# glennhickey/teHmm

Hardware: AMD Instinct MI355X
Metric: genome positions/sec (Viterbi+posterior), 35 states x 10 tracks (higher is better)
Workload: dtype f64

## Files before the change

### tehmm_amd/csrc/tehmm_coop.hip.h

```cpp
#pragma once
#include "tehmm_kernels.hip.h"

namespace tehmm {

typedef double d2v __attribute__((ext_vector_type(2)));
typedef __attribute__((address_space(3))) const d2v lds_cd2;
__device__ __forceinline__ lds_cd2 *lds_row(const double *row) {
  unsigned a = (unsigned)(size_t)(__attribute__((address_space(3))) const double *)row;
  asm volatile("v_mov_b32 %0, %1" : "=v"(a) : "v"(a));
  return (lds_cd2 *)(size_t)a;
}

template <int NT>
__device__ __forceinline__ void rep_rows(double v, double (&r)[(NT + 15) / 16]) {
  const unsigned lo = __double2loint(v), hi = __double2hiint(v);
  const auto a = __builtin_amdgcn_permlane32_swap(lo, lo, false, false);
  const auto b = __builtin_amdgcn_permlane32_swap(hi, hi, false, false);
  const auto c = __builtin_amdgcn_permlane16_swap(a[0], a[0], false, false);
  const auto d = __builtin_amdgcn_permlane16_swap(b[0], b[0], false, false);
  r[0] = __hiloint2double((int)d[0], (int)c[0]);
  if constexpr (NT > 16) r[1] = __hiloint2double((int)d[1], (int)c[1]);
  if constexpr (NT > 32) {
    const auto e = __builtin_amdgcn_permlane16_swap(a[1], a[1], false, false);
    const auto f = __builtin_amdgcn_permlane16_swap(b[1], b[1], false, false);
    r[2] = __hiloint2double((int)f[0], (int)e[0]);
    if constexpr (NT > 48) r[3] = __hiloint2double((int)f[1], (int)e[1]);
  }
}
template <int L>
__device__ __forceinline__ double bcast(double v) {
  return __longlong_as_double(
      __builtin_amdgcn_mov_dpp(__double_as_longlong(v), 0x150 + L, 0xf, 0xf, true));
}
template <int F, int NT>
struct BcastAdd {
  static __device__ __forceinline__ void run(const double (&r)[(NT + 15) / 16], const double (&ltc)[NT],
                                             double (&x)[NT]) {
    x[F] = bcast<F & 15>(r[F >> 4]) + ltc[F];
    BcastAdd<F + 1, NT>::run(r, ltc, x);
  }
};
template <int NT>
struct BcastAdd<NT, NT> {
  static __device__ __forceinline__ void run(const double (&)[(NT + 15) / 16], const double (&)[NT],
                                             double (&)[NT]) {}
};
template <int F, int NT>
struct BcastFma {
  static __device__ __forceinline__ void run(const double (&r)[(NT + 15) / 16], const double (&ac)[NT],
                                             double (&s)[4]) {
    asm volatile("v_fmac_f64_dpp %0, %1, %2 row_newbcast:%3 row_mask:0xf bank_mask:0xf"
                 : "+v"(s[F & 3])
                 : "v"(r[F >> 4]), "v"(ac[F]), "n"(F & 15));
    BcastFma<F + 1, NT>::run(r, ac, s);
  }
};
template <int NT>
struct BcastFma<NT, NT> {
  static __device__ __forceinline__ void run(const double (&)[(NT + 15) / 16], const double (&)[NT],
                                             double (&)[4]) {}
};

__device__ __forceinline__ double exp_nonpos(double y) {
  const double k = rint(y * 1.4426950408889634);
  double r = fma(k, -6.93147180369123816490e-01, y);
  r = fma(k, -1.90821492927058770002e-10, r);
  double p = 1.6059043836821613e-10;
  p = fma(p, r, 2.08767569878681e-09);
  p = fma(p, r, 2.505210838544172e-08);
  p = fma(p, r, 2.755731922398589e-07);
  p = fma(p, r, 2.7557319223985893e-06);
  p = fma(p, r, 2.48015873015873e-05);
  p = fma(p, r, 1.984126984126984e-04);
  p = fma(p, r, 1.388888888888889e-03);
  p = fma(p, r, 8.333333333333333e-03);
  p = fma(p, r, 4.1666666666666664e-02);
  p = fma(p, r, 1.6666666666666666e-01);
  p = fma(p, r, 0.5);
  p = fma(p, r, 1.0);
  p = fma(p, r, 1.0);
  const double res = ldexp(p, (int)k);
  return y < -1100.0 ? 0.0 : res;
}

template <int NT>
__device__ __forceinline__ void emis_rows(const EmisTab &e, const double *ltab, int64_t gpos,
                                          double (&x)[NT]) {
  const uint32_t *row = e.obs32 + gpos * e.KPW;
#pragma unroll
  for (int j = 0; j < NT; ++j) x[j] = 0.0;
  uint32_t wn = row[0];
  for (int d = 0; d < e.KPW; ++d) {
    const uint32_t w = wn;
    if (d + 1 < e.KPW) wn = row[d + 1];
#pragma unroll
    for (int bb = 0; bb < 4; ++bb) {
      const int k = 4 * d + bb;
      if (k < e.K) {
        const int sym = (int)((w >> (8 * bb)) & 0xffu);
        const bool inr = sym < e.rowcnt[k];
        const int lb = e.ldsbase[k];
        if (lb >= 0) {
          lds_cd2 *tr = (lds_cd2 *)(size_t)((unsigned)(size_t)(
              __attribute__((address_space(3))) const double *)ltab +
              (unsigned)((inr ? lb + sym : e.lds_zero) * NT * 8));
#pragma unroll
          for (int jj = 0; jj < NT / 2; ++jj) {
            const d2v v = tr[jj];
            x[2 * jj] += v.x;
            x[2 * jj + 1] += v.y;
          }
        } else {
          const double2 *tr = (const double2 *)(e.tab + (int64_t)(inr ? e.rowbase[k] + sym : e.zero_row) * NT);
#pragma unroll
          for (int jj = 0; jj < NT / 2; ++jj) {
            const double2 v = tr[jj];
            x[2 * jj] += v.x;
            x[2 * jj + 1] += v.y;
          }
        }
      }
    }
  }
#pragma unroll
  for (int j = 0; j < NT; ++j) x[j] *= e.normalize;
  if (e.ratios) {
    const double r = e.ratios[gpos];
#pragma unroll
    for (int j = 0; j < NT; ++j) x[j] *= r;
  }
}

template <int NT, bool LINEAR, bool ASCENDING, bool TRATIO>
__device__ __forceinline__ void emis_block(const EmisTab &e, const double *ltab, int64_t gbase,
                                           int np, int lane, int N, bool &seen, int *dead,
                                           const double *ltdiag, const double *tratios,
                                           double *ring, int RS, double *ms) {
  const bool act = lane < np;
  const int64_t gpos = gbase + (act ? lane : np - 1);
  double x[NT];
  emis_rows<NT>(e, ltab, gpos, x);
  double m = x[0];
#pragma unroll
  for (int j = 1; j < NT; ++j) m = fmax(m, j < N ? x[j] : -INFINITY);
  const bool good = m > -1e20;
  bool zero;
  if (ASCENDING) {
    const unsigned long long gm = __ballot(good && act);
    const int first = gm ? __ffsll((long long)gm) - 1 : 64;
    zero = !seen && lane < first;
    if (!good && !zero && act && dead) *dead = 1;
    if (gm) seen = true;
  } else {
    zero = !good;
  }
  if (zero) {
#pragma unroll
    for (int j = 0; j < NT; ++j) x[j] = 0.0;
    m = 0.0;
  }
  if (TRATIO) {
    const double r = tratios[gpos];
    if (r > 1.) {
      m = -INFINITY;
#pragma unroll
      for (int j = 0; j < NT; ++j) {
        x[j] += ltdiag[j] * (r - 1.);
        m = fmax(m, j < N ? x[j] : -INFINITY);
      }
    }
  }
  if (act) {
    double *dst = ring + lane * RS;
    if (LINEAR) {
#pragma unroll
      for (int j = 0; j < NT; ++j) dst[j] = j < N ? exp_nonpos(x[j] - m) : 0.0;
      ms[lane] = m;
    } else {
#pragma unroll
      for (int j = 0; j < NT; ++j) dst[j] = x[j];
    }
  }
}

__device__ __forceinline__ void stage_emis_table(const EmisTab &e, double *ltab, int NT) {
  const int n = e.lds_rows * NT;
  for (int i = threadIdx.x; i < n; i += blockDim.x) ltab[i] = e.ltab_src[i];
}

template <int NT, int CPB, bool RATIO>
__global__ __launch_bounds__(256) __attribute__((amdgpu_waves_per_eu(1, 1)))
void k_vit_coop(IntervalTab iv, EmisTab em, int N, const double *g_lt, const double *g_ltT,
                const double *g_pi, const double *tratios, uint8_t *tb, int *last_state, double *logprob) {
  extern __shared__ double sm[];
  constexpr int RS = NT + 1;
  constexpr int VS = NT + 2;
  double *bring = sm;
  double *Vring = bring + 3 * CPB * RS;
  double *ltab = Vring + 2 * (CPB + 1) * VS;
  const int lane = threadIdx.x & 63;
  const int w = threadIdx.x >> 6;
  const int id = iv.order[blockIdx.x];
  const int64_t T = iv.len[id];
  const int64_t p0 = iv.pos0[id];
  if (T <= 0) return;
  stage_emis_table(em, ltab, NT);
  const int jl = min(lane, NT - 1);
  const bool live = lane < N;
  ST_DECL;
  __syncthreads();
  const int64_t nb = (T + CPB - 1) / CPB;
  if (w == 0) {
    double ltc[NT];
#pragma unroll
    for (int f = 0; f < NT; ++f) ltc[f] = live ? g_lt[f * NT + jl] : -INFINITY;
    const double ltd = live ? g_lt[jl * NT + jl] : 0.0;
    const double lt00 = g_lt[0];
    const double pij = live ? g_pi[jl] : -INFINITY;
    const int vslot = lane < NT ? lane : NT + 1;
    double vcur = -INFINITY;
    for (int64_t it = 0; it < nb + 2; ++it) {
      ST_BEGIN;
      const int64_t bn = it - 1;
      if (bn >= 0 && bn < nb) {
        const int np = (int)min((int64_t)CPB, T - bn * CPB);
        double *Vr = Vring + (bn & 1) * (CPB + 1) * VS;
        const double *br = bring + (bn % 3) * CPB * RS;
        if (bn > 0) Vr[vslot] = vcur;
        for (int p = 0; p < np; ++p) {
          const int64_t t = bn * CPB + p;
          const double b = br[p * RS + jl];
          double r = 0.0;
          if (RATIO) r = tratios[p0 + t];
          double v;
          if (t == 0) {
            v = pij + b;
            if (RATIO && r > 1.) v += ltd * (r - 1.);
          } else {
            double rr[(NT + 15) / 16];
            rep_rows<NT>(vcur, rr);
            double x[NT];
            BcastAdd<0, NT>::run(rr, ltc, x);
            double c0 = x[0] + b;
            x[0] = -INFINITY;
#pragma unroll
            for (int n = NT; n > 1; n = (n + 1) / 2) {
#pragma unroll
              for (int i = 0; i < n / 2; ++i) x[i] = fmax(x[i], x[i + (n + 1) / 2]);
            }
            if (RATIO) {
              c0 += ltd * r;
              if (lane == 0) c0 -= lt00;
            }
            double c1 = x[0] + b;
            if (RATIO && r > 1.) c1 += ltd * (r - 1.);
            v = c1 > c0 ? c1 : c0;
          }
          vcur = v;
          Vr[(p + 1) * VS + vslot] = v;
        }
      }
      ST_ADD(st_a);
      __syncthreads();
      ST_ADD(st_c);
    }
    ST_FLUSH(w);
    double *scratch = Vring;
    if (lane < NT) scratch[lane] = vcur;
    __builtin_amdgcn_wave_barrier();
    if (lane == 0) {
      int last = 0;
      double m = scratch[0];
      if (m == m) {
        for (int j = 1; j < N; ++j) {
          double x = scratch[j];
          if (x != x) { last = j; break; }
          if (x > m) { m = x; last = j; }
        }
      }
      last_state[id] = last;
      logprob[id] = scratch[last];
    }
  } else if (w == 1) {
    bool seen = false;
    for (int64_t it = 0; it < nb + 2; ++it) {
      ST_BEGIN;
#ifdef TEHMM_DBG_NOEMIS
      if (it < 3) {
#else
      if (it < nb) {
#endif
        const int np = (int)min((int64_t)CPB, T - it * CPB);
        emis_block<NT, false, true, false>(em, ltab, p0 + it * CPB, np, lane, N, seen, nullptr,
                                           nullptr, nullptr, bring + (it % 3) * CPB * RS, RS,
                                           nullptr);
      }
      ST_ADD(st_a);
      __syncthreads();
      ST_ADD(st_c);
    }
    ST_FLUSH(w);
  } else {
    const int half = (N + 1) / 2;
    const int to_lo = (w - 2) * half, to_hi = min(N, to_lo + half);
    const double lt00 = g_lt[0];
    for (int64_t it = 0; it < nb + 2; ++it) {
      ST_BEGIN;
      const int64_t ba = it - 2;
#ifdef TEHMM_DBG_NOARGS
      if (ba >= 0 && ba < 1) {
#else
      if (ba >= 0 && ba < nb) {
#endif
        const int np = (int)min((int64_t)CPB, T - ba * CPB);
        const double *Vr = Vring + (ba & 1) * (CPB + 1) * VS;
        const double *br = bring + (ba % 3) * CPB * RS;
        const int pl = lane < np ? lane : 0;
        const int64_t t = ba * CPB + pl;
        const bool actp = lane < np && t > 0;
        lds_cd2 *vp = lds_row(Vr + pl * VS);
        d2v pv[NT / 2];
#pragma unroll
        for (int f2 = 0; f2 < NT / 2; ++f2) pv[f2] = vp[f2];
        const double *vnext = Vr + (pl + 1) * VS;
        const double *brow = br + pl * RS;
        double r = 0.0;
        if (RATIO) r = tratios[p0 + t];
        const bool rg = RATIO && r > 1.;
        for (int to = to_lo; to < to_hi; ++to) {
          const double *lc = g_ltT + to * NT;
          const double vt = vnext[to];
          const double b = brow[to];
          double c[NT];
#pragma unroll
          for (int f2 = 0; f2 < NT / 2; ++f2) {
            c[2 * f2] = (pv[f2].x + lc[2 * f2]) + b;
            c[2 * f2 + 1] = (pv[f2].y + lc[2 * f2 + 1]) + b;
          }
          if (RATIO) {
            const double ld = lc[to];
            c[0] += ld * r;
            if (to == 0) c[0] -= lt00;
            const double addr = rg ? ld * (r - 1.) : 0.0;
#pragma unroll
            for (int f = 1; f < NT; ++f) c[f] += addr;
          }
          int arg = 0;
#pragma unroll
          for (int f = NT - 1; f >= 1; --f) arg = c[f] == vt ? f : arg;
          arg = c[0] == vt ? 0 : arg;
          if (actp) tb[(p0 + t) * NT + to] = (uint8_t)arg;
        }
      }
      ST_ADD(st_b);
      __syncthreads();
      ST_ADD(st_c);
    }
    ST_FLUSH(w);
  }
}

template <int NT, int CPB, bool TRATIO>
__global__ __launch_bounds__(256) __attribute__((amdgpu_waves_per_eu(1, 1)))
void k_fb_coop(IntervalTab iv, EmisTab em, int N, const double *g_A, const double *g_lt,
               const double *g_pi, const double *tratios, double *alpha, double *beta,
               double *fwd_logprob, int *dead_flag, double *wrows, int *escale) {
  extern __shared__ double sm[];
  constexpr int RS = NT + 1;
  double *ringF = sm;
  double *ringB = ringF + 2 * CPB * RS;
  double *msF = ringB + 2 * CPB * RS;
  double *msB = msF + 2 * CPB;
  double *xF = msB + 2 * CPB;
  double *xB = xF + 2 * NT;
  double *ltdv = xB + 2 * NT;
  double *ltab = ltdv + NT;
  const int lane = threadIdx.x & 63;
  const int w = threadIdx.x >> 6;
  const int id = iv.order[blockIdx.x];
  const int64_t T = iv.len[id];
  const int64_t p0 = iv.pos0[id];
  if (T <= 0) return;
  const int jl = min(lane, NT - 1);
  const bool live = lane < N;
  if (threadIdx.x < NT) ltdv[threadIdx.x] = g_lt[threadIdx.x * NT + threadIdx.x];
  stage_emis_table(em, ltab, NT);
  ST_DECL;
  __syncthreads();
  const int64_t nb = (T + CPB - 1) / CPB;
  if (w == 0) {
    double ac[NT];
#pragma unroll
    for (int i = 0; i < NT; ++i) ac[i] = live ? g_A[i * NT + jl] : (lane == NT - 1 ? 1.0 : 0.0);
    double *al = alpha + iv.out0[id] * N;
    int *es = escale ? escale + iv.out0[id] : nullptr;
    double Ecum = 0.0, Mcum = 0.0, a = 0.0;
    for (int64_t it = 0; it < nb + 1; ++it) {
      ST_BEGIN;
      const int64_t bn = it - 1;
      if (bn >= 0) {
        const int np = (int)min((int64_t)CPB, T - bn * CPB);
        const double *br = ringF + (bn & 1) * CPB * RS;
        const double *mr = msF + (bn & 1) * CPB;
        for (int p = 0; p < np; ++p) {
          const int64_t t = bn * CPB + p;
          const double bh = br[p * RS + jl];
          Mcum += mr[p];
          if (t == 0) {
            a = live ? exp(g_pi[jl]) * bh : 0.0;
          } else {
            double rr[(NT + 15) / 16];
            rep_rows<NT>(a, rr);
            double sacc[4] = {0.0, 0.0, 0.0, 0.0};
            asm volatile("s_nop 1" ::: "memory");
            BcastFma<0, NT>::run(rr, ac, sacc);
            const double ssum = (sacc[0] + sacc[1]) + (sacc[2] + sacc[3]);
            const int e = ((__builtin_amdgcn_readlane(__double2hiint(ssum), NT - 1) >> 20) & 0x7ff) - 1022;
            a = live ? ldexp(ssum * bh, -e) : 0.0;
            Ecum += (double)e;
            if (es && lane == 0) es[t] = e;
          }
          if (live) al[t * N + lane] = a;
        }
      }
      ST_ADD(st_a);
      __syncthreads();
      ST_ADD(st_c);
    }
    ST_FLUSH(w);
    double tot = wave_sum_f64(live ? a : 0.0);
    if (lane == 0) fwd_logprob[id] = log(tot) + Ecum * 0.6931471805599453 + Mcum;
  } else if (w == 1) {
    double ac[NT];
#pragma unroll
    for (int j = 0; j < NT; ++j) ac[j] = live ? g_A[jl * NT + j] : (lane == NT - 1 ? 1.0 : 0.0);
    double *be = beta + iv.out0[id] * N;
    double *wr = wrows ? wrows + iv.out0[id] * N : nullptr;
    double bt = 0.0, wv = 0.0;
    for (int64_t it = 0; it < nb + 1; ++it) {
      ST_BEGIN;
      const int64_t bn = it - 1;
      if (bn >= 0) {
        const int64_t uhi = T - bn * CPB;
        const int64_t ulo = max((int64_t)0, uhi - CPB);
        const double *br = ringB + (bn & 1) * CPB * RS;
        for (int64_t u = uhi - 1; u >= ulo; --u) {
          const double bh = br[(int)(u - ulo) * RS + jl];
          if (u == T - 1) {
            bt = live ? 1.0 : 0.0;
          } else {
            double rr[(NT + 15) / 16];
            rep_rows<NT>(wv, rr);
            double sacc[4] = {0.0, 0.0, 0.0, 0.0};
            asm volatile("s_nop 1" ::: "memory");
            BcastFma<0, NT>::run(rr, ac, sacc);
            const double ssum = (sacc[0] + sacc[1]) + (sacc[2] + sacc[3]);
            const int e = ((__builtin_amdgcn_readlane(__double2hiint(ssum), NT - 1) >> 20) & 0x7ff) - 1022;
            bt = live ? ldexp(ssum, -e) : 0.0;
          }
          if (live) be[u * N + lane] = bt;
          wv = live ? bh * bt : 0.0;
          if (wr && live) wr[u * N + lane] = wv;
        }
      }
      ST_ADD(st_a);
      __syncthreads();
      ST_ADD(st_c);
    }
    ST_FLUSH(w);
  } else if (w == 2) {
    bool seen = false;
    for (int64_t it = 0; it < nb + 1; ++it) {
      ST_BEGIN;
      if (it < nb) {
        const int np = (int)min((int64_t)CPB, T - it * CPB);
        emis_block<NT, true, true, TRATIO>(em, ltab, p0 + it * CPB, np, lane, N, seen, dead_flag + id,
                                           ltdv, tratios, ringF + (it & 1) * CPB * RS, RS,
                                           msF + (it & 1) * CPB);
      }
      ST_ADD(st_a);
      __syncthreads();
      ST_ADD(st_c);
    }
    ST_FLUSH(w);
  } else {
    for (int64_t it = 0; it < nb + 1; ++it) {
      ST_BEGIN;
      if (it < nb) {
        const int64_t uhi = T - it * CPB;
        const int64_t ulo = max((int64_t)0, uhi - CPB);
// ... 200 lines not shown
```

### tehmm_amd/csrc/tehmm_lane.hip.h

```cpp
#pragma once
#include "tehmm_spec.hip.h"

namespace tehmm {

typedef __attribute__((address_space(4))) const double const_f64;
#define TEHMM_TG(f, o, NT) ((((o) >> 2) * (NT) + (f)) * 4 + ((o) & 3))



template <int NT>
__global__ __launch_bounds__(256) void k_emis_lane(IntervalTab iv, EmisTab em, LaneGeom lg, int N,
                                                   double *B, double *BH, double *MS, float *B32) {
  extern __shared__ double emis_ltab[];
  stage_emis_table(em, emis_ltab, NT);
  __syncthreads();
  const int lane = threadIdx.x & 63;
  const int g = blockIdx.x * 4 + (threadIdx.x >> 6);
  if (g >= lg.n_groups) return;
  const int64_t item = (int64_t)g * 64 + lane;
  const bool valid = item < lg.n_items;
  const int id = valid ? lg.item_iv[item] : 0;
  const int64_t t0 = valid ? lg.item_t0[item] : 0;
  const int64_t T = iv.len[id], p0 = iv.pos0[id];
  const int len = valid ? (int)min((int64_t)lg.L, T - t0) : 0;
// ... 663 lines not shown
    vec_out(vi.end);
    if (QUANT) {
      vi.ntie[item] = nt;
      vi.bad[item] = (bad || nt > TEHMM_LANE_MAXTI) ? 1 : 0;
      vi.piecemin[item * (TEHMM_LANE_MAXTI + 1) + min(nt, TEHMM_LANE_MAXTI)] = pmin;
    } else {
      const double g1 = vec_max();
      vi.gain[item] = bad ? __longlong_as_double(0x7ff8000000000000LL) : g1 - g0;
    }
  }
}

template <int NT>
__global__ __launch_bounds__(256) void k_vit_stitch(IntervalTab iv, LaneGeom lg, VitChunks vc, VitItems vi,
                                                    int N, int soft = 0) {
  const int lane = threadIdx.x & 63;
  const int c = blockIdx.x * 4 + (threadIdx.x >> 6);
  if (c >= vc.n) return;
  if (vc.e[c] == TEHMM_SPEC_NONE) {
    if (lane == 0) { vc.ok[c] = 0; vc.ntie[c] = 0; vc.offend[c] = 0.0; if (vc.tsoft) { vc.tsoft[c] = 0u; vc.tpar[c] = 0u; } }
    return;
  }
  unsigned softmask = 0u, parmask = 0u;
  const double uinv = ldexp(1.0, 52 - vc.e[c]);
  auto odd_mult = [&](double x) { const double q = x * uinv * 0.5; return q != trunc(q); };
  const int id = vc.iv[c];
  const int64_t ct0 = vc.t0[c];
  const int L = lg.L, SUB = vc.CS / L, R = L / TEHMM_VROW;
  const int64_t item0 = lg.ifirst[id] + ct0 / L;
  const bool live = lane < N;
  const int jl = min(lane, NT - 1);
  auto at = [&](const double *p, int64_t item) { return p[((((item >> 6) * NT) + jl) << 6) + (item & 63)]; };
  double off = 0.0, off_end = 0.0, segmin = INFINITY;
  int nT = 0;
  bool okc = true;
  for (int k = 0; k < SUB; ++k) {
    const int64_t item = item0 + k;
    okc = okc && vi.bad[item] == 0;
    off = off_end;
    if (k > 0) {
      const double a = at(vi.pre, item), bp = at(vi.end, item - 1);
      const bool both_dead = a == -INFINITY && bp == -INFINITY;
      const double d = bp - a;
      const double d0 = wave_max_live((both_dead || !live) ? -INFINITY : d, live);
      const bool same = __all(!live || both_dead || d == d0) && d0 == d0 && d0 > -INFINITY && d0 < INFINITY;
      if (same) {
        off = off_end + d0;
      } else {
        if (nT < TEHMM_SPEC_MAXT) {
          if (lane == 0) {
            vc.ties[(int64_t)c * TEHMM_SPEC_MAXT + nT] = k * L;
            vc.segmin[(int64_t)c * (TEHMM_SPEC_MAXT + 1) + nT] = segmin;
          }
          if (lane < NT) vc.tierows[((int64_t)c * TEHMM_SPEC_MAXT + nT) * NT + lane] = bp + off_end;
        }
        ++nT;
        off = 0.0;
        segmin = INFINITY;
      }
    }
    const int nti = min(vi.ntie[item], TEHMM_LANE_MAXTI);
    const int first_tie = nti > 0 ? vi.ties[item * TEHMM_LANE_MAXTI] : L;
    if (off != 0.0 && lane < NT) {
      for (int m = 0; m < R && (soft || TEHMM_VROW * m + TEHMM_VROW - 1 < first_tie); ++m)
        vc.rows[((int64_t)c * (vc.CS / TEHMM_VROW) + k * R + m) * NT + lane] += off;
    }
    segmin = fmin(segmin, vi.piecemin[item * (TEHMM_LANE_MAXTI + 1)] + off);
    for (int i = 0; i < nti; ++i) {
      if (nT < TEHMM_SPEC_MAXT) {
        if (lane == 0) {
          vc.ties[(int64_t)c * TEHMM_SPEC_MAXT + nT] = k * L + vi.ties[item * TEHMM_LANE_MAXTI + i];
          vc.segmin[(int64_t)c * (TEHMM_SPEC_MAXT + 1) + nT] = segmin;
        }
        if (lane < NT)
          vc.tierows[((int64_t)c * TEHMM_SPEC_MAXT + nT) * NT + lane] =
              vi.tierows[(item * TEHMM_LANE_MAXTI + i) * NT + lane] + ((i == 0 || soft) ? off : 0.0);
        if (soft) {
          softmask |= 1u << nT;
          if (odd_mult(off)) parmask |= 1u << nT;
        }
      }
      ++nT;
      segmin = vi.piecemin[item * (TEHMM_LANE_MAXTI + 1) + i + 1] + (soft ? off : 0.0);
    }
    off_end = (nti > 0 && !soft) ? 0.0 : off;
  }
  if (lane == 0) {
    vc.segmin[(int64_t)c * (TEHMM_SPEC_MAXT + 1) + min(nT, TEHMM_SPEC_MAXT)] = segmin;
    vc.ntie[c] = nT;
    vc.ok[c] = (okc && nT <= TEHMM_SPEC_MAXT) ? 1 : 0;
    vc.offend[c] = off_end;
    if (vc.tsoft) { vc.tsoft[c] = softmask; vc.tpar[c] = parmask; }
  }
}

template <int NT>
__global__ __launch_bounds__(256) void k_vit_links(IntervalTab iv, LaneGeom lg, VitChunks vc, VitItems vi, int N) {
  const int lane = threadIdx.x & 63;
  const int c = blockIdx.x * 4 + (threadIdx.x >> 6);
  if (c >= vc.n) return;
  const int id = vc.iv[c];
  bool cand = c > vc.first[id] && vc.e[c] != TEHMM_SPEC_NONE && vc.e[c - 1] == vc.e[c] && vc.ok[c] != 0 &&
              vc.ok[c - 1] != 0;
  int link = 0;
  double lk = 0.0;
  if (cand) {
    const int L = lg.L;
    const int64_t item0 = lg.ifirst[id] + vc.t0[c] / L;
    const bool live = lane < N;
    const int jl = min(lane, NT - 1);
    auto at = [&](const double *p, int64_t item) { return p[((((item >> 6) * NT) + jl) << 6) + (item & 63)]; };
    const double a = at(vi.pre, item0);
    const double bp = at(vi.end, item0 - 1) + vc.offend[c - 1];
    const bool both_dead = a == -INFINITY && bp == -INFINITY;
    const double d = bp - a;
    const double d0 = wave_max_live((both_dead || !live) ? -INFINITY : d, live);
    const bool same = __all(!live || both_dead || d == d0) && d0 == d0 && d0 > -INFINITY && d0 < INFINITY;
    if (same && vi.bad[item0 - 1] == 0 && vi.bad[item0] == 0) {
      link = 1;
      lk = d0;
    }
  }
  if (lane == 0) {
    vc.clink[c] = link;
    vc.clk[c] = lk;
  }
}


struct VitRunMap {
  int stop;
  int64_t target, sel;
  double acc, mn;
};
struct VitRunMap2 {
  VitRunMap m[2];
  int hout[2];
};
__device__ __forceinline__ VitRunMap2 vit_run_compose(const VitRunMap2 &a, const VitRunMap2 &b) {
  VitRunMap2 r;
#pragma unroll
  for (int h = 0; h < 2; ++h) {
    if (a.m[h].stop) {
      r.m[h] = a.m[h];
      r.hout[h] = 0;
    } else {
      const int h2 = a.hout[h];
      const VitRunMap &bb = h2 ? b.m[1] : b.m[0];
      r.m[h].stop = bb.stop;
      r.m[h].target = bb.target;
      r.m[h].sel = bb.sel;
      r.m[h].acc = a.m[h].acc + bb.acc;
      r.m[h].mn = fmin(a.m[h].mn, a.m[h].acc + bb.mn);
      r.hout[h] = h2 ? b.hout[1] : b.hout[0];
    }
  }
  return r;
}
__global__ __launch_bounds__(64) void k_vit_runs(VitChunks vc, int n_iv) {
  const int lane = threadIdx.x;
  const int id = blockIdx.x;
  if (id >= n_iv) return;
  const int64_t c0 = vc.first[id], c1 = vc.first[id + 1];
  const int64_t nc = vc.n;
  VitRunMap2 carry;
  carry.m[0] = carry.m[1] = VitRunMap{0, 0, 0, 0.0, INFINITY};
  carry.hout[0] = 0;
  carry.hout[1] = 1;
  for (int64_t hi = c1; hi > c0; hi -= 64) {
    const int64_t c = hi - 64 + lane;
    const bool in = c >= c0;
    VitRunMap2 m;
    m.m[0] = m.m[1] = VitRunMap{0, 0, 0, 0.0, INFINITY};
    m.hout[0] = 0;
    m.hout[1] = 1;
    if (in) {
      const double *sm = vc.segmin + c * (TEHMM_SPEC_MAXT + 1);
      const bool linked_next = c + 1 < c1 && vc.clink[c + 1] != 0;
      const int nt = min(vc.ntie[c], TEHMM_SPEC_MAXT);
      const unsigned soft = vc.tsoft ? vc.tsoft[c] : 0u, par = vc.tsoft ? vc.tpar[c] : 0u;
      int kodd = 0;
      if (linked_next) {
        const double q = vc.clk[c + 1] * ldexp(1.0, 52 - vc.e[c]) * 0.5;
        kodd = q != trunc(q);
      }
#pragma unroll
      for (int h = 0; h < 2; ++h) {
        int kh = -1;
        double mn = sm[0];
        for (int k = 0; k < nt; ++k) {
          if (!((soft >> k) & 1u) || (int)((par >> k) & 1u) != h) { kh = k; break; }
          mn = fmin(mn, sm[k + 1]);
        }
        if (kh >= 0) m.m[h] = VitRunMap{1, vc.t0[c] + vc.ties[c * TEHMM_SPEC_MAXT + kh], 2 * (64 * c + kh), 0.0, mn};
        else if (linked_next) m.m[h] = VitRunMap{0, 0, 0, vc.clk[c + 1], mn};
        else m.m[h] = VitRunMap{1, vc.t0[c] + vc.CS, 2 * (64 * c) + 1, 0.0, mn};
        m.hout[h] = h ^ kodd;
      }
    }
#pragma unroll
    for (int d = 1; d < 64; d <<= 1) {
      VitRunMap2 o;
#pragma unroll
      for (int h = 0; h < 2; ++h) {
        o.m[h].stop = __shfl_down(m.m[h].stop, d);
        o.m[h].target = __shfl_down(m.m[h].target, d);
        o.m[h].sel = __shfl_down(m.m[h].sel, d);
        o.m[h].acc = __shfl_down(m.m[h].acc, d);
        o.m[h].mn = __shfl_down(m.m[h].mn, d);
        o.hout[h] = __shfl_down(m.hout[h], d);
      }
      if (lane + d < 64) m = vit_run_compose(m, o);
    }
    m = vit_run_compose(m, carry);
    if (in) {
#pragma unroll
      for (int h = 0; h < 2; ++h) {
        vc.rtarget[h * nc + c] = m.m[h].target;
        vc.rsel[h * nc + c] = m.m[h].sel;
        vc.racc[h * nc + c] = m.m[h].acc;
        vc.rmn[h * nc + c] = m.m[h].mn;
      }
    }
#pragma unroll
    for (int h = 0; h < 2; ++h) {
      carry.m[h].stop = __shfl(m.m[h].stop, 0);
      carry.m[h].target = __shfl(m.m[h].target, 0);
      carry.m[h].sel = __shfl(m.m[h].sel, 0);
      carry.m[h].acc = __shfl(m.m[h].acc, 0);
      carry.m[h].mn = __shfl(m.m[h].mn, 0);
      carry.hout[h] = __shfl(m.hout[h], 0);
    }
  }
}


typedef float lane_f2 __attribute__((ext_vector_type(2)));
typedef __attribute__((address_space(4))) const lane_f2 const_f2;

template <int NT>
__global__ __launch_bounds__(256) void k_vit_gain_lane(IntervalTab iv, LaneGeom lg, int N, int CS, int Wu,
                                                       const float *__restrict__ tabf,
                                                       const float *__restrict__ B32, double *gain) {
  const int lane = threadIdx.x & 63;
  const int g = blockIdx.x * 4 + (threadIdx.x >> 6);
  if (g >= lg.n_groups) return;
  const int L = lg.L;
  const int64_t item = (int64_t)g * 64 + lane;
  const bool valid = item < lg.n_items;
  const int id = valid ? lg.item_iv[item] : 0;
  const int64_t t0 = valid ? lg.item_t0[item] : 0;
  const int64_t T = iv.len[id];
  const int64_t ct0 = (t0 / CS) * CS;
  const bool run = valid && ct0 > 0 && ct0 + CS <= T;
  if (!__any(run)) return;
  const int64_t nb = run ? item - 1 : item;
  lane_f2 W[NT / 2];
#pragma unroll
  for (int j = 0; j < NT / 2; ++j)
    W[j] = (lane_f2){2 * j < N ? 0.f : -INFINITY, 2 * j + 1 < N ? 0.f : -INFINITY};
  bool bad = false;
  auto vec_max = [&]() {
    float mx = -INFINITY;
#pragma unroll
    for (int j = 0; j < NT / 2; ++j) mx = fmaxf(mx, fmaxf(W[j].x, W[j].y));
    return mx;
  };
  float g0 = 0.f;
  for (int s = -Wu; s < L; ++s) {
    if (s == 0) g0 = vec_max();
    const float *bp = B32 + (s < 0 ? lane_row(lg, NT, nb, L + s) : lane_row(lg, NT, item, s));
    float b[NT];
#pragma unroll
    for (int j = 0; j < NT; ++j) b[j] = bp[(int64_t)j << 6];
    bad = bad | (b[0] != b[0]);
    int z = 0;
    asm volatile("" : "+s"(z));
    const_f2 *tp = (const_f2 *)(size_t)tabf + z;
    lane_f2 x[NT / 2];
#pragma unroll
    for (int op = 0; op < NT / 2; ++op) {
      lane_f2 acc = (lane_f2){W[0].x, W[0].x} + tp[op * NT];
#pragma unroll
      for (int f = 1; f < NT; ++f) {
        const float wf = (f & 1) ? W[f >> 1].y : W[f >> 1].x;
        acc = __builtin_elementwise_max(acc, (lane_f2){wf, wf} + tp[op * NT + f]);
      }
      x[op] = acc;
    }
#pragma unroll
    for (int j = 0; j < NT / 2; ++j) W[j] = x[j] + (lane_f2){b[2 * j], b[2 * j + 1]};
  }
  if (run) gain[item] = bad ? __longlong_as_double(0x7ff8000000000000LL) : (double)vec_max() - (double)g0;
}

template <int NT, bool RATIO = false>
#ifndef TEHMM_EMIS_WAVES
#define TEHMM_EMIS_WAVES 2
#endif
__global__ __launch_bounds__(256) __attribute__((amdgpu_waves_per_eu(TEHMM_EMIS_WAVES, TEHMM_EMIS_WAVES))) void k_emis_gain_lane(IntervalTab iv, EmisTab em, LaneGeom lg, int N, int CS, int Wu,
                                                        const float *__restrict__ tabf, double *B, double *gain,
                                                        const double *__restrict__ ratios = nullptr) {
  extern __shared__ double emis_ltab[];
  stage_emis_table(em, emis_ltab, NT);
  __syncthreads();
  const int lane = threadIdx.x & 63;
  const int g = blockIdx.x * 4 + (threadIdx.x >> 6);
  if (g >= lg.n_groups) return;
  const int L = lg.L;
  const int64_t item = (int64_t)g * 64 + lane;
  const bool valid = item < lg.n_items;
  const int id = valid ? lg.item_iv[item] : 0;
  const int64_t t0 = valid ? lg.item_t0[item] : 0;
  const int64_t T = iv.len[id], p0 = iv.pos0[id];
  const int len = valid ? (int)min((int64_t)L, T - t0) : 0;
  const int maxlen = wave_max_i32(len);
  const int64_t ct0 = (t0 / CS) * CS;
  const bool run = valid && ct0 > 0 && ct0 + CS <= T;
  const int s_first = __any(run) ? -Wu : 0;
  const double qnan = __longlong_as_double(0x7ff8000000000000LL);
  lane_f2 W[NT / 2];
#pragma unroll
  for (int j = 0; j < NT / 2; ++j)
    W[j] = (lane_f2){2 * j < N ? 0.f : -INFINITY, 2 * j + 1 < N ? 0.f : -INFINITY};
  bool bad = false;
  auto vec_max = [&]() {
    float mx = -INFINITY;
#pragma unroll
    for (int j = 0; j < NT / 2; ++j) mx = fmaxf(mx, fmaxf(W[j].x, W[j].y));
    return mx;
  };
  float g0 = 0.f;
  for (int s = s_first; s < maxlen; ++s) {
    const bool act = s >= 0 ? s < len : run;
    const int64_t gpos = p0 + t0 + (act ? s : 0);
    double x[NT];
    emis_rows<NT>(em, emis_ltab, gpos, x);
    double m = x[0];
#pragma unroll
    for (int j = 1; j < NT; ++j) m = fmax(m, j < N ? x[j] : -INFINITY);
    const bool good = m > -1e20;
    if (B && s >= 0 && act) {
      const int64_t o = ((((int64_t)g * lg.L + s) * NT) << 6) + lane;
#pragma unroll
      for (int j = 0; j < NT; ++j) B[o + ((int64_t)j << 6)] = good ? x[j] : qnan;
    }
    if (s == 0) g0 = vec_max();
    bad = bad | (act && !good);
    int z = 0;
    asm volatile("" : "+s"(z));
    const_f2 *tp = (const_f2 *)(size_t)tabf + z;
    lane_f2 xn[NT / 2];
    float rf = 1.f, rm1 = 0.f;
    if (RATIO) {
      rf = (float)ratios[gpos];
      rm1 = rf > 1.f ? rf - 1.f : 0.f;
    }
#pragma unroll
    for (int op = 0; op < NT / 2; ++op) {
      lane_f2 acc = (lane_f2){W[0].x, W[0].x} + tp[op * NT];
      if (RATIO) {
        const lane_f2 ltd = tp[NT * NT / 2 + op];
        acc = acc + ltd * (lane_f2){rf - rm1, rf - rm1};
        if (op == 0) acc.x -= ((const float *)(size_t)tabf)[z + NT * NT + NT];
      }
#pragma unroll
      for (int f = 1; f < NT; ++f) {
        const float wf = (f & 1) ? W[f >> 1].y : W[f >> 1].x;
        acc = __builtin_elementwise_max(acc, (lane_f2){wf, wf} + tp[op * NT + f]);
      }
      xn[op] = acc;
    }
#pragma unroll
    for (int j = 0; j < NT / 2; ++j) {
      W[j] = xn[j] + (lane_f2){(float)x[2 * j], (float)x[2 * j + 1]};
      if (RATIO) W[j] = W[j] + tp[NT * NT / 2 + j] * (lane_f2){rm1, rm1};
    }
  }
  if (run) gain[item] = (bad || len < L) ? qnan : (double)vec_max() - (double)g0;
}

}
```

Before: 1.489 billion.

## Add precomputed emission program with prefetched observation words in gain kernel

Precomputes a per-track emission program (row base, count, zero row, LDS/global flag) in shared memory, then replaces the generic emis_rows lookup in k_emis_gain_lane with a loop driven by that program. Observation words for the next position are loaded one step ahead so their latency overlaps the current position's work. The B store also skips the NaN select when no active lane in the wave is bad. This adds shared memory, registers and a wave vote, and the program path only covers up to 16 tracks.

```diff
diff --git a/tehmm_amd/csrc/tehmm_coop.hip.h b/tehmm_amd/csrc/tehmm_coop.hip.h
--- a/tehmm_amd/csrc/tehmm_coop.hip.h
+++ b/tehmm_amd/csrc/tehmm_coop.hip.h
@@ -186,6 +186,73 @@
 __device__ __forceinline__ void stage_emis_table(const EmisTab &e, double *ltab, int NT) {
   const int n = e.lds_rows * NT;
   for (int i = threadIdx.x; i < n; i += blockDim.x) ltab[i] = e.ltab_src[i];
+}
+
+#define TEHMM_EMIS_PROG_KPW 4
+__device__ __forceinline__ void stage_emis_prog(const EmisTab &e, const double *ltab, int4 *prog, int NT) {
+  const unsigned lbase = (unsigned)(size_t)(__attribute__((address_space(3))) const double *)ltab;
+  const int k = threadIdx.x;
+  if (k < e.K && k < 4 * TEHMM_EMIS_PROG_KPW) {
+    const int lb = e.ldsbase[k];
+    int4 p;
+    p.x = lb >= 0 ? (int)(lbase + (unsigned)(lb * NT * 8)) : e.rowbase[k] * NT * 8;
+    p.y = e.rowcnt[k];
+    p.z = lb >= 0 ? (int)(lbase + (unsigned)(e.lds_zero * NT * 8)) : e.zero_row * NT * 8;
+    p.w = lb >= 0 ? 1 : 0;
+    prog[k] = p;
+  }
+}
+
+template <int NT>
+__device__ __forceinline__ void emis_rows_prog(const EmisTab &e, const int4 *prog, uint32_t (&w)[TEHMM_EMIS_PROG_KPW],
+                                               bool norm1, int64_t gpos, double (&x)[NT]) {
+#pragma unroll
+  for (int j = 0; j < NT; ++j) x[j] = 0.0;
+  const int K = e.K;
+  int4 pn = prog[0];
+  for (int k = 0; k < K; ++k) {
+    const int row0 = __builtin_amdgcn_readfirstlane(pn.x), cnt = __builtin_amdgcn_readfirstlane(pn.y);
+    const int zrow = __builtin_amdgcn_readfirstlane(pn.z), in_lds = __builtin_amdgcn_readfirstlane(pn.w);
+    pn = prog[k + 1 < K ? k + 1 : k];
+    const int sym = (int)(w[0] & 0xffu);
+#pragma unroll
+    for (int d = 0; d + 1 < TEHMM_EMIS_PROG_KPW; ++d) w[d] = __builtin_amdgcn_alignbyte(w[d + 1], w[d], 1);
+    w[TEHMM_EMIS_PROG_KPW - 1] >>= 8;
+    const int off = sym < cnt ? row0 + sym * (NT * 8) : zrow;
+    double t[NT];
+    if (in_lds) {
+      lds_cd2 *tr = (lds_cd2 *)(size_t)(unsigned)off;
+#pragma unroll
+      for (int jj = 0; jj < NT / 2; ++jj) {
+        const d2v v = tr[jj];
+        t[2 * jj] = v.x;
+        t[2 * jj + 1] = v.y;
+      }
+    } else {
+      const double2 *tr = (const double2 *)((const char *)e.tab + off);
+#pragma unroll
+      for (int jj = 0; jj < NT / 2; ++jj) {
+        const double2 v = tr[jj];
+        t[2 * jj] = v.x;
+        t[2 * jj + 1] = v.y;
+      }
+    }
+#pragma unroll
+    for (int jj = 0; jj < NT / 2; ++jj) {
+      asm volatile("" : "+v"(t[2 * jj]), "+v"(t[2 * jj + 1]));
+      x[2 * jj] += t[2 * jj];
+      x[2 * jj + 1] += t[2 * jj + 1];
+    }
+  }
+  if (!norm1) {
+#pragma unroll
+    for (int j = 0; j < NT; ++j) x[j] *= e.normalize;
+  }
+  if (e.ratios) {
+    const double r = e.ratios[gpos];
+#pragma unroll
+    for (int j = 0; j < NT; ++j) x[j] *= r;
+  }
 }
 
 template <int NT, int CPB, bool RATIO>
diff --git a/tehmm_amd/csrc/tehmm_lane.hip.h b/tehmm_amd/csrc/tehmm_lane.hip.h
--- a/tehmm_amd/csrc/tehmm_lane.hip.h
+++ b/tehmm_amd/csrc/tehmm_lane.hip.h
@@ -989,8 +989,12 @@
                                                         const float *__restrict__ tabf, double *B, double *gain,
                                                         const double *__restrict__ ratios = nullptr) {
   extern __shared__ double emis_ltab[];
+  __shared__ int4 emis_prog[4 * TEHMM_EMIS_PROG_KPW];
   stage_emis_table(em, emis_ltab, NT);
+  stage_emis_prog(em, emis_ltab, emis_prog, NT);
   __syncthreads();
+  const bool use_prog = NT <= 40 && em.KPW <= TEHMM_EMIS_PROG_KPW;
+  const bool norm1 = em.normalize == 1.0;
   const int lane = threadIdx.x & 63;
   const int g = blockIdx.x * 4 + (threadIdx.x >> 6);
   if (g >= lg.n_groups) return;
@@ -1018,19 +1022,47 @@
     return mx;
   };
   float g0 = 0.f;
+  uint32_t wn[TEHMM_EMIS_PROG_KPW];
+  auto request_words = [&](int s) {
+    const bool a = s >= 0 ? s < len : run;
+    const uint32_t *row = em.obs32 + (p0 + t0 + (a ? s : 0)) * em.KPW;
+#pragma unroll
+    for (int d = 0; d < TEHMM_EMIS_PROG_KPW; ++d) wn[d] = d < em.KPW ? row[d] : 0u;
+  };
+#pragma unroll
+  for (int d = 0; d < TEHMM_EMIS_PROG_KPW; ++d) wn[d] = 0u;
+  if (use_prog && s_first < maxlen) request_words(s_first);
   for (int s = s_first; s < maxlen; ++s) {
     const bool act = s >= 0 ? s < len : run;
     const int64_t gpos = p0 + t0 + (act ? s : 0);
     double x[NT];
-    emis_rows<NT>(em, emis_ltab, gpos, x);
+    if (use_prog) {
+      uint32_t w[TEHMM_EMIS_PROG_KPW];
+#pragma unroll
+      for (int d = 0; d < TEHMM_EMIS_PROG_KPW; ++d) {
+        asm volatile("" : "+v"(wn[d]));
+        w[d] = wn[d];
+      }
+      emis_rows_prog<NT>(em, emis_prog, w, norm1, gpos, x);
+      if (s + 1 < maxlen) request_words(s + 1);
+    } else {
+      emis_rows<NT>(em, emis_ltab, gpos, x);
+    }
     double m = x[0];
 #pragma unroll
     for (int j = 1; j < NT; ++j) m = fmax(m, j < N ? x[j] : -INFINITY);
     const bool good = m > -1e20;
-    if (B && s >= 0 && act) {
+    if (B && s >= 0) {
       const int64_t o = ((((int64_t)g * lg.L + s) * NT) << 6) + lane;
-#pragma unroll
-      for (int j = 0; j < NT; ++j) B[o + ((int64_t)j << 6)] = good ? x[j] : qnan;
+      if (__any(act && !good)) {
+        if (act) {
+#pragma unroll
+          for (int j = 0; j < NT; ++j) B[o + ((int64_t)j << 6)] = good ? x[j] : qnan;
+        }
+      } else if (act) {
+#pragma unroll
+        for (int j = 0; j < NT; ++j) B[o + ((int64_t)j << 6)] = x[j];
+      }
     }
     if (s == 0) g0 = vec_max();
     bad = bad | (act && !good);
```

Result: no change. 1.500 billion (median of 6 runs) (+0.7%).
